# varunbachalli/PoseEstimationKF

Measured on AMD Instinct MI355X. Metric: EKF steps/sec (predict+Wahba+update) at batch=1M; HBM-roofline %, higher is better.
Workload: dtype f64

## Files before the change

### poseestimationkf_amd/csrc/pekf_math.hpp

```cpp
#pragma once

#include <hip/hip_runtime.h>

#include <cmath>
#include <cstdint>
#include <type_traits>

#define PEKF_DEV __device__ __forceinline__

#ifdef PEKF_ISA_COMMON_PATH
#define PEKF_TAKEN(cond, common) (common)
#else
#define PEKF_TAKEN(cond, common) __builtin_expect(!!(cond), 0)
#endif

namespace pekf {

constexpr double kNsToS = 1e-09;
constexpr double kSqrt2 = 1.4142135623730951;


PEKF_DEV void omega_half(const double *w, double *A) {
    A[0] = 0.0;          A[1] = -0.5 * w[0];  A[2] = -0.5 * w[1];  A[3] = -0.5 * w[2];
    A[4] = 0.5 * w[0];   A[5] = 0.0;          A[6] = 0.5 * w[2];   A[7] = -0.5 * w[1];
// ... 303 lines not shown
}

template <int FAST>
PEKF_DEV void wahba_current_rank1(const double *acc0, const double *mag0, const double *acc, const double *mag,
                                  double ka, double km, double *R) {
    double v[3], w[3];
    current_rank1_directions<FAST>(acc0, mag0, acc, mag, ka, km, v, w);
    shortest_arc<FAST>(v, w, R);
}

template <int FAST>
PEKF_DEV void wahba_current_rank1_quat(const double *acc0, const double *mag0, const double *acc, const double *mag,
                                       double ka, double km, double *q) {
    double v[3], w[3], n[3];
    current_rank1_directions<FAST>(acc0, mag0, acc, mag, ka, km, v, w);
    const double c1 = fma(v[0], w[0], fma(v[1], w[1], fma(v[2], w[2], 1.0)));
    const double k[3] = {v[1] * w[2] - v[2] * w[1], v[2] * w[0] - v[0] * w[2], v[0] * w[1] - v[1] * w[0]};
    normal_of(v, n);
    const bool half = !(c1 * c1 + k[0] * k[0] + k[1] * k[1] + k[2] * k[2] > 0.0) && (w[0] == w[0]);
    const double t[4] = {half ? 0.0 : c1, half ? n[0] : k[0], half ? n[1] : k[1], half ? n[2] : k[2]};
    const double it = rsqrt<FAST>(t[0] * t[0] + t[1] * t[1] + t[2] * t[2] + t[3] * t[3]);
    q[0] = t[0] * it; q[1] = t[1] * it; q[2] = t[2] * it; q[3] = t[3] * it;
}

PEKF_DEV void frame_pair(const Frame &F, double *a, double *m) {
#pragma unroll
    for (int i = 0; i < 3; ++i) {
        a[i] = F.alpha * F.e1[i];
        m[i] = F.beta1 * F.e1[i] + F.beta2 * F.e2[i];
    }
}

PEKF_DEV void wahba_rotation_vectors(const double *acc0, const double *mag0, const double *acc,
                                     const double *mag, double ka, double km, double *R) {
    Frame W, V;
    make_frame(acc0, mag0, W);
    make_frame(acc, mag, V, wahba_sign(ka, km));
    if (frame_degenerate(W) || frame_degenerate(V))
        wahba_rank1_rotation(acc0, mag0, acc, mag, ka, km, R);
    else
        wahba_rotation(W, V, ka, km, R);
}

PEKF_DEV void rotm_to_quat_scaled(const double *M, double *v, double &inv_s) {
    const double t1 = ((1.0 + M[0]) - M[4]) - M[8];
    const double t2 = ((1.0 - M[0]) + M[4]) - M[8];
    const double t3 = ((1.0 - M[0]) - M[4]) + M[8];
    const bool b1 = (t1 > t2) && (t1 > t3);
    const bool b2 = !b1 && (t2 > t1) && (t2 > t3);
    const bool b3 = !b1 && !b2;
    const double t = b1 ? t1 : (b2 ? t2 : t3);
    inv_s = 0.5 * rsqrt<true>(t);
    const double dw1 = M[7] - M[5], dw2 = M[2] - M[6], dw3 = M[3] - M[1];
    const double sxy = M[1] + M[3], sxz = M[2] + M[6], syz = M[5] + M[7];
    v[0] = b1 ? dw1 : (b2 ? dw2 : dw3);
    v[1] = b1 ? t : (b2 ? sxy : sxz);
    v[2] = b2 ? t : (b1 ? sxy : syz);
    v[3] = b3 ? t : (b1 ? sxz : syz);
}

PEKF_DEV void rotm_to_quat_fast(const double *M, double *q) {
    double v[4], inv_s;
    rotm_to_quat_scaled(M, v, inv_s);
    q[0] = v[0] * inv_s; q[1] = v[1] * inv_s; q[2] = v[2] * inv_s; q[3] = v[3] * inv_s;
}

PEKF_DEV void q4_times(const double *M, const double *z, double *v, double &nv, double &t0) {
    const double a = 1.0 + M[8], b = 1.0 - M[8], s = M[0] + M[4], d = M[0] - M[4];
    t0 = a + s;
    const double t1 = b + d, t2 = b - d, t3 = a - s;
    const double dw1 = M[7] - M[5], dw2 = M[2] - M[6], dw3 = M[3] - M[1];
    const double sxy = M[1] + M[3], sxz = M[2] + M[6], syz = M[5] + M[7];
    v[0] = fma(t0, z[0], fma(dw1, z[1], fma(dw2, z[2], dw3 * z[3])));
    v[1] = fma(dw1, z[0], fma(t1, z[1], fma(sxy, z[2], sxz * z[3])));
    v[2] = fma(dw2, z[0], fma(sxy, z[1], fma(t2, z[2], syz * z[3])));
    v[3] = fma(dw3, z[0], fma(sxz, z[1], fma(syz, z[2], t3 * z[3])));
    nv = fma(v[0], v[0], fma(v[1], v[1], fma(v[2], v[2], v[3] * v[3])));
}

PEKF_DEV void rotm_to_quat_flip_reference(const double *M, const double *z, double *v, double &sc) {
    double inv_s;
    rotm_to_quat_scaled(M, v, inv_s);
    const double cmp = v[0] * z[0] + v[1] * z[1] + v[2] * z[2] + v[3] * z[3];
    sc = cmp < 0.0 ? -inv_s : inv_s;
}

PEKF_DEV void rotm_to_quat_toward(const double *M, const double *z, double *v, double &sc) {
    double nv, t0;
    q4_times(M, z, v, nv, t0);
    sc = rsqrt<true>(nv);
    if (PEKF_TAKEN(nv < 1.0 || t0 > 4.0 - 1e-10, false))
        rotm_to_quat_flip_reference(M, z, v, sc);
}

struct RefW {
    static constexpr bool kRefBasis = true;
    double aW, b1W, b2W;
    double q[4];
    PEKF_DEV void quat(double *o) const { o[0] = q[0]; o[1] = q[1]; o[2] = q[2]; o[3] = q[3]; }
};

PEKF_DEV void frame_quat(const Frame &F, double *q) {
    const double m00 = F.e1[0], m10 = F.e1[1], m20 = F.e1[2];
    const double m01 = F.e2[0], m11 = F.e2[1], m21 = F.e2[2];
    const double m02 = F.u3[0], m12 = F.u3[1], m22 = F.u3[2];
    const double t0 = 1.0 + m00 + m11 + m22, t1 = 1.0 + m00 - m11 - m22;
    const double t2 = 1.0 - m00 + m11 - m22, t3 = 1.0 - m00 - m11 + m22;
    const double w1 = m21 - m12, w2 = m02 - m20, w3 = m10 - m01;
    const double sxy = m01 + m10, sxz = m02 + m20, syz = m12 + m21;
    double v0, v1, v2, v3;
    if (t0 >= t1 && t0 >= t2 && t0 >= t3) {
        v0 = t0; v1 = w1; v2 = w2; v3 = w3;
    } else if (t1 >= t2 && t1 >= t3) {
        v0 = w1; v1 = t1; v2 = sxy; v3 = sxz;
    } else if (t2 >= t3) {
        v0 = w2; v1 = sxy; v2 = t2; v3 = syz;
    } else {
        v0 = w3; v1 = sxz; v2 = syz; v3 = t3;
    }
    const double in = 1.0 / sqrt(v0 * v0 + v1 * v1 + v2 * v2 + v3 * v3);
    q[0] = v0 * in; q[1] = v1 * in; q[2] = v2 * in; q[3] = v3 * in;
}

struct RefWLazy {
    static constexpr bool kRefBasis = true;
    double aW, b1W, b2W;
    const double *pair;
    PEKF_DEV void quat(double *o) const {
        Frame F;
        make_frame<true>(pair, pair + 3, F);
        frame_quat(F, o);
    }
};

template <bool CONJ>
PEKF_DEV void qmul_left(const double *q, const double *x, double *y) {
    const double q0 = q[0], q1 = CONJ ? -q[1] : q[1], q2 = CONJ ? -q[2] : q[2], q3 = CONJ ? -q[3] : q[3];
    y[0] = q0 * x[0] - q1 * x[1] - q2 * x[2] - q3 * x[3];
    y[1] = q0 * x[1] + q1 * x[0] + q2 * x[3] - q3 * x[2];
    y[2] = q0 * x[2] - q1 * x[3] + q2 * x[0] + q3 * x[1];
    y[3] = q0 * x[3] + q1 * x[2] - q2 * x[1] + q3 * x[0];
}

PEKF_DEV void quat_to_rotm(const double *q, double *M) {
    const double w = q[0], x = q[1], y = q[2], z = q[3];
    M[0] = 1.0 - 2.0 * (y * y + z * z); M[1] = 2.0 * (x * y - w * z);       M[2] = 2.0 * (x * z + w * y);
    M[3] = 2.0 * (x * y + w * z);       M[4] = 1.0 - 2.0 * (x * x + z * z); M[5] = 2.0 * (y * z - w * x);
    M[6] = 2.0 * (x * z - w * y);       M[7] = 2.0 * (y * z + w * x);       M[8] = 1.0 - 2.0 * (x * x + y * y);
}

struct NoPin {
    PEKF_DEV void operator()() const {}
};
template <int F = 1, class RW, std::enable_if_t<RW::kRefBasis, int> = 0>
PEKF_DEV void wahba_rotation_ref(const RW &W, const Frame &V, double ka, double km, double *R) {
    const double kw = km * W.b2W, kb = km * W.b1W;
    double p = ka * W.aW * V.alpha + kb * V.beta1 + kw * V.beta2;
    double s = kw * V.beta1 - kb * V.beta2;
    const double ih = rsqrt<F>(p * p + s * s);
    p *= ih;
    s *= ih;
#pragma unroll
    for (int j = 0; j < 3; ++j) {
        R[j] = p * V.e1[j] - s * V.e2[j];
        R[3 + j] = s * V.e1[j] + p * V.e2[j];
        R[6 + j] = V.u3[j];
    }
}

template <int F = 1, class RW, class Reload, class Pin = NoPin, std::enable_if_t<RW::kRefBasis, int> = 0>
PEKF_DEV void wahba_toward_from_rotation(const RW &W, const double *R, const double *z, double *v, double &sc,
                                         const Reload &reload, const Pin &pin = Pin()) {
    double nv, t0;
    q4_times(R, z, v, nv, t0);
    sc = rsqrt<F>(nv);
    pin();
    if (PEKF_TAKEN(!(nv >= 1.0), false)) {
        double Fw[9], Rw[9], zw[4], vw[4], qw[4];
        W.quat(qw);
        quat_to_rotm(qw, Fw);
#pragma unroll
        for (int i = 0; i < 3; ++i)
#pragma unroll
            for (int j = 0; j < 3; ++j) Rw[3 * i + j] = Fw[3 * i] * R[j] + Fw[3 * i + 1] * R[3 + j] + Fw[3 * i + 2] * R[6 + j];
        qmul_left<false>(qw, z, zw);
        rotm_to_quat_flip_reference(Rw, zw, vw, sc);
        qmul_left<true>(qw, vw, v);
        if (!(nv == nv)) {
            double acc[3], mag[3];
            reload(acc, mag);
            const double a0[3] = {W.aW, 0.0, 0.0}, m0[3] = {W.b1W, W.b2W, 0.0}, kr = fabs(acc[2]);
            wahba_current_rank1_quat<1>(a0, m0, acc, mag, kr, 1.0 - kr, v);
            sc = v[0] * z[0] + v[1] * z[1] + v[2] * z[2] + v[3] * z[3] < 0.0 ? -1.0 : 1.0;
        }
    }
    (void)t0;
}

template <int F = 1, class RW, class Reload, class Pin = NoPin, std::enable_if_t<RW::kRefBasis, int> = 0>
PEKF_DEV void wahba_quat_toward(const RW &W, const Frame &V, double ka, double km, const double *z, double *v,
                                double &sc, const Reload &reload, const Pin &pin = Pin()) {
    const double kw = km * W.b2W, kb = km * W.b1W;
    double p = ka * W.aW * V.alpha + kb * V.beta1 + kw * V.beta2;
    double s = kw * V.beta1 - kb * V.beta2;
    const double ih = rsqrt<F>(p * p + s * s);
    p *= ih;
    s *= ih;
    double R[9];
#pragma unroll
    for (int j = 0; j < 3; ++j) {
        R[j] = p * V.e1[j] - s * V.e2[j];
        R[3 + j] = s * V.e1[j] + p * V.e2[j];
        R[6 + j] = V.u3[j];
    }
    double nv, t0;
    q4_times(R, z, v, nv, t0);
    sc = rsqrt<F>(nv);
    pin();
    if (PEKF_TAKEN(!(nv >= 1.0), false)) {
        double Fw[9], Rw[9], zw[4], vw[4], qw[4];
        W.quat(qw);
        quat_to_rotm(qw, Fw);
#pragma unroll
        for (int i = 0; i < 3; ++i)
#pragma unroll
            for (int j = 0; j < 3; ++j) Rw[3 * i + j] = Fw[3 * i] * R[j] + Fw[3 * i + 1] * R[3 + j] + Fw[3 * i + 2] * R[6 + j];
        qmul_left<false>(qw, z, zw);
        rotm_to_quat_flip_reference(Rw, zw, vw, sc);
        qmul_left<true>(qw, vw, v);
        if (!(nv == nv)) {
            double acc[3], mag[3];
            reload(acc, mag);
            const double a0[3] = {W.aW, 0.0, 0.0}, m0[3] = {W.b1W, W.b2W, 0.0}, kr = fabs(acc[2]);
            wahba_current_rank1_quat<1>(a0, m0, acc, mag, kr, 1.0 - kr, v);
            sc = v[0] * z[0] + v[1] * z[1] + v[2] * z[2] + v[3] * z[3] < 0.0 ? -1.0 : 1.0;
        }
    }
    (void)t0;
}

template <int F = 1, class Reload, class Pin = NoPin>
PEKF_DEV void wahba_quat_toward(const Frame &W, const Frame &V, double ka, double km, const double *z, double *v,
                                double &sc, const Reload &reload, const Pin & = Pin()) {
    double R[9], nv, t0;
    wahba_rotation<true>(W, V, ka, km, R);
    q4_times(R, z, v, nv, t0);
    sc = rsqrt<true>(nv);
    if (PEKF_TAKEN(!(nv >= 1.0) || t0 > 4.0 - 1e-10, false)) {
        rotm_to_quat_flip_reference(R, z, v, sc);
        if (!(nv == nv)) {
            double acc[3], mag[3], a0[3], m0[3];
            reload(acc, mag);
            frame_pair(W, a0, m0);
            const double kr = fabs(acc[2]);
            wahba_current_rank1_quat<1>(a0, m0, acc, mag, kr, 1.0 - kr, v);
            sc = v[0] * z[0] + v[1] * z[1] + v[2] * z[2] + v[3] * z[3] < 0.0 ? -1.0 : 1.0;
        }
    }
}


template <typename T>
struct Sym4T {
    T a00, a01, a02, a03, a11, a12, a13, a22, a23, a33;
};
using Sym4 = Sym4T<double>;

template <bool CONJ, typename T>
PEKF_DEV Sym4T<T> sym_rotate(const double *q, const Sym4T<T> &S) {
    const double p[4][4] = {{S.a00, S.a01, S.a02, S.a03}, {S.a01, S.a11, S.a12, S.a13},
                            {S.a02, S.a12, S.a22, S.a23}, {S.a03, S.a13, S.a23, S.a33}};
    double t[4][4], o[4][4];
#pragma unroll
    for (int j = 0; j < 4; ++j) {
        double c[4];
        qmul_left<CONJ>(q, p[j], c);
#pragma unroll
        for (int i = 0; i < 4; ++i) t[i][j] = c[i];
    }
#pragma unroll
    for (int i = 0; i < 4; ++i) qmul_left<CONJ>(q, t[i], o[i]);
    return {(T)o[0][0], (T)o[0][1], (T)o[0][2], (T)o[0][3], (T)o[1][1],
            (T)o[1][2], (T)o[1][3], (T)o[2][2], (T)o[2][3], (T)o[3][3]};
}

template <bool FAST>
PEKF_DEV float recip(float x) {
    if (!FAST) return 1.0f / x;
    float r = __builtin_amdgcn_rcpf(x);
    return fmaf(r, fmaf(-x, r, 1.0f), r);
}

template <typename T>
PEKF_DEV Sym4T<T> innovation_cov2(const Sym4T<T> &P, const T *h, const T *w, T th2, const T *x, T n2, T g2, T r2,
                                  T g2x) {
    const T sp = P.a00 + P.a11, dp = P.a11 - P.a00, sq = P.a22 + P.a33, dq = P.a22 - P.a33;
    const T tr = sp + sq, d11 = sq - sp, d22 = dp - dq, d33 = dp + dq;
    const T u0 = fma(d11, h[0], fma(P.a03 - P.a12, w[1], -(P.a02 + P.a13) * w[2]));
    const T u1 = fma(d22, h[1], fma(P.a01 - P.a23, w[2], -(P.a03 + P.a12) * w[0]));
    const T u2 = fma(d33, h[2], fma(P.a02 - P.a13, w[0], -(P.a01 + P.a23) * w[1]));
    const T uh = fma(u0, h[0], fma(u1, h[1], u2 * h[2]));
    const T c0 = fma(u1, h[2], -u2 * h[1]), c1 = fma(u2, h[0], -u0 * h[2]);
    const T c2 = fma(u0, h[1], -u1 * h[0]);
    const T nt = T(-2) * th2;
    const T base = fma(th2, tr, fma(g2, n2, r2));
    const T b0 = base - uh, bk = base + uh;
    const T gx0 = g2x * x[0], gx1 = g2x * x[1], gx2 = g2x * x[2], gx3 = g2x * x[3];
    Sym4T<T> o;
    o.a00 = fma(nt, P.a00, fma(-gx0, x[0], b0));
    o.a01 = fma(nt, P.a01, fma(-gx0, x[1], c0));
    o.a02 = fma(nt, P.a02, fma(-gx0, x[2], c1));
    o.a03 = fma(nt, P.a03, fma(-gx0, x[3], c2));
    o.a11 = fma(nt, P.a11, fma(-gx1, x[1], fma(-u0, w[0], bk)));
    o.a22 = fma(nt, P.a22, fma(-gx2, x[2], fma(-u1, w[1], bk)));
    o.a33 = fma(nt, P.a33, fma(-gx3, x[3], fma(-u2, w[2], bk)));
    o.a12 = fma(nt, P.a12, fma(-gx1, x[2], -fma(u0, h[1], u1 * h[0])));
    o.a13 = fma(nt, P.a13, fma(-gx1, x[3], -fma(u0, h[2], u2 * h[0])));
    o.a23 = fma(nt, P.a23, fma(-gx2, x[3], -fma(u1, h[2], u2 * h[1])));
    return o;
}

template <typename T>
PEKF_DEV Sym4T<T> innovation_cov_n(const Sym4T<T> &N, const T *h, const T *w, T th2, const T *x, T n2, T gb, T rb,
                                   T gbx) {
    const T sp = N.a00 + N.a11, dp = N.a11 - N.a00, sq = N.a22 + N.a33, dq = N.a22 - N.a33;
    const T tr = sp + sq, d11 = sq - sp, d22 = dp - dq, d33 = dp + dq;
    const T u0 = fma(d11, h[0], fma(N.a12 - N.a03, w[1], (N.a02 + N.a13) * w[2]));
    const T u1 = fma(d22, h[1], fma(N.a01 - N.a23, w[2], (N.a03 + N.a12) * w[0]));
    const T u2 = fma(d33, h[2], fma(N.a13 - N.a02, w[0], -(N.a01 + N.a23) * w[1]));
    const T uh = fma(u0, h[0], fma(u1, h[1], u2 * h[2]));
    const T c0 = fma(u1, h[2], -u2 * h[1]), c1 = fma(u2, h[0], -u0 * h[2]);
    const T c2 = fma(u0, h[1], -u1 * h[0]);
    const T nt = T(-2) * th2;
    const T base = fma(th2, tr + rb, fma(gb, n2, rb));
    const T b0 = base - uh, bk = base + uh;
    const T gx0 = gbx * x[0], gx1 = gbx * x[1], gx2 = gbx * x[2], gx3 = gbx * x[3];
    Sym4T<T> o;
    o.a00 = fma(nt, N.a00, fma(-gx0, x[0], b0));
    o.a01 = fma(nt, N.a01, fma(-gx0, x[1], c0));
    o.a02 = fma(-nt, N.a02, fma(-gx0, x[2], c1));
    o.a03 = fma(-nt, N.a03, fma(-gx0, x[3], c2));
    o.a11 = fma(nt, N.a11, fma(-gx1, x[1], fma(-u0, w[0], bk)));
    o.a22 = fma(nt, N.a22, fma(-gx2, x[2], fma(-u1, w[1], bk)));
    o.a33 = fma(nt, N.a33, fma(-gx3, x[3], fma(-u2, w[2], bk)));
    o.a12 = fma(-nt, N.a12, fma(-gx1, x[2], -fma(u0, h[1], u1 * h[0])));
    o.a13 = fma(-nt, N.a13, fma(-gx1, x[3], -fma(u0, h[2], u2 * h[0])));
    o.a23 = fma(nt, N.a23, fma(-gx2, x[3], -fma(u1, h[2], u2 * h[1])));
    return o;
}

PEKF_DEV Sym4 innovation_cov_n_w(const Sym4 &N, const double *w, double th2x2, const double *x, double n2, double gb,
                                 double rb, double rbh, double gbx) {
    const double sp = N.a00 + N.a11, dp = N.a11 - N.a00, sq = N.a22 + N.a33, dq = N.a22 - N.a33;
    const double trh = add_half(sp, sq) + rbh;
    const double d11h = sub_half(sq, sp), d22h = sub_half(dp, dq), d33h = add_half(dp, dq);
    const double u0 = fma(d11h, w[0], fma(N.a12 - N.a03, w[1], (N.a02 + N.a13) * w[2]));
    const double u1 = fma(d22h, w[1], fma(N.a01 - N.a23, w[2], (N.a03 + N.a12) * w[0]));
    const double u2 = fma(d33h, w[2], fma(N.a13 - N.a02, w[0], -(N.a01 + N.a23) * w[1]));
    const double uh = fma_half(u0, w[0], fma(u1, w[1], u2 * w[2]));
    const double c0 = fma_half_nc(u1, w[2], u2 * w[1]), c1 = fma_half_nc(u2, w[0], u0 * w[2]);
    const double c2 = fma_half_nc(u0, w[1], u1 * w[0]);
    const double base = fma(th2x2, trh, fma(gb, n2, rb));
    const double b0 = base - uh, bk = base + uh;
    const double gx0 = gbx * x[0], gx1 = gbx * x[1], gx2 = gbx * x[2], gx3 = gbx * x[3];
    Sym4 o;
    o.a00 = fma(-th2x2, N.a00, fma(-gx0, x[0], b0));
    o.a01 = fma(-th2x2, N.a01, fma(-gx0, x[1], c0));
    o.a02 = fma(th2x2, N.a02, fma(-gx0, x[2], c1));
    o.a03 = fma(th2x2, N.a03, fma(-gx0, x[3], c2));
    o.a11 = fma(-th2x2, N.a11, fma(-gx1, x[1], fma(-u0, w[0], bk)));
    o.a22 = fma(-th2x2, N.a22, fma(-gx2, x[2], fma(-u1, w[1], bk)));
    o.a33 = fma(-th2x2, N.a33, fma(-gx3, x[3], fma(-u2, w[2], bk)));
    o.a12 = fma(th2x2, N.a12, fma(-gx1, x[2], -fma_half(u0, w[1], u1 * w[0])));
    o.a13 = fma(th2x2, N.a13, fma(-gx1, x[3], -fma_half(u0, w[2], u2 * w[0])));
    o.a23 = fma(-th2x2, N.a23, fma(-gx2, x[3], -fma_half(u1, w[2], u2 * w[1])));
    return o;
}

template <typename T, bool FAST = true, bool NEG = false>
PEKF_DEV Sym4T<T> spd_inverse_schur(const Sym4T<T> &S) {
    const T ia = recip<FAST>(S.a00 * S.a11 - S.a01 * S.a01);
    const T p00 = S.a11 * ia, p01 = -S.a01 * ia, p11 = S.a00 * ia;
    const T x00 = p00 * S.a02 + p01 * S.a12, x01 = p00 * S.a03 + p01 * S.a13;
    const T x10 = p01 * S.a02 + p11 * S.a12, x11 = p01 * S.a03 + p11 * S.a13;
    const T c00 = S.a22 - S.a02 * x00 - S.a12 * x10;
    const T c01 = S.a23 - S.a02 * x01 - S.a12 * x11;
    const T c11 = S.a33 - S.a03 * x01 - S.a13 * x11;
    const T ic = NEG ? recip<FAST>(c01 * c01 - c00 * c11) : recip<FAST>(c00 * c11 - c01 * c01);
    const T q00 = c11 * ic, q01 = -c01 * ic, q11 = c00 * ic;
    Sym4T<T> o;
    if (NEG) {
// ... 67 lines not shown
```

### poseestimationkf_amd/csrc/pekf_step.hpp

```cpp
#pragma once

#include <type_traits>

#include "pekf_internal.hpp"
#include "pekf_math.hpp"
#include "pekf_tile.hpp"

namespace pekf {

constexpr int kRunBlock = 256;

#ifndef PEKF_REC_AUX
#define PEKF_REC_AUX 2
#endif

template <bool SOA, typename PT>
__device__ __forceinline__ void load_state(const double *X, const double *P, int64_t b, int64_t batch,
                                           double *x, Sym4T<PT> &S) {
    if (SOA) {
#pragma unroll
        for (int k = 0; k < 4; ++k) x[k] = X[k * batch + b];
        S = {(PT)P[0 * batch + b], (PT)P[1 * batch + b], (PT)P[2 * batch + b], (PT)P[3 * batch + b],
             (PT)P[4 * batch + b], (PT)P[5 * batch + b], (PT)P[6 * batch + b], (PT)P[7 * batch + b],
             (PT)P[8 * batch + b], (PT)P[9 * batch + b]};
// ... 40 lines not shown

    __device__ __forceinline__ RowCursor(const float4 *gd, const float4 *am, const float2 *my, int64_t batch,
                                         int64_t win)
        : g(reinterpret_cast<const char *>(gd)), a(reinterpret_cast<const char *>(am)),
          m(reinterpret_cast<const char *>(my)), row16((uint32_t)batch * 16u), row8((uint32_t)batch * 8u),
          window((int32_t)win) {
        const uint32_t c = (1u << 31) / row16;
        chunk_rows = c ? (int32_t)c : 1;
    }
    __device__ __forceinline__ void start(int32_t r) {
        row = r;
        end = (window - r < chunk_rows) ? window : r + chunk_rows;
        const uint64_t n = (uint64_t)(end - r);
        rg = row_rsrc(g + (uint64_t)r * row16, (int64_t)(n * row16));
        ra = row_rsrc(a + (uint64_t)r * row16, (int64_t)(n * row16));
        rm = row_rsrc(m + (uint64_t)r * row8, (int64_t)(n * row8));
        s16 = 0;
        s8 = 0;
    }
    __device__ __forceinline__ void advance() {
        if (++row == end) {
            start(row == window ? 0 : row);
        } else {
            s16 += row16;
            s8 += row8;
        }
    }
    __device__ __forceinline__ Rec load(uint32_t off16, uint32_t off8) const {
        Rec v;
        v.gd = __builtin_bit_cast(float4, __builtin_amdgcn_raw_buffer_load_b128(rg, off16, s16, PEKF_REC_AUX));
        v.am = __builtin_bit_cast(float4, __builtin_amdgcn_raw_buffer_load_b128(ra, off16, s16, PEKF_REC_AUX));
        v.my = __builtin_bit_cast(float2, __builtin_amdgcn_raw_buffer_load_b64(rm, off8, s8, PEKF_REC_AUX));
        return v;
    }
};

template <typename PT>
__device__ __forceinline__ Sym4T<PT> sym_from16(const double (&p)[16]) {
    return {(PT)p[0], (PT)p[1], (PT)p[2], (PT)p[3], (PT)p[5], (PT)p[6], (PT)p[7], (PT)p[10], (PT)p[11], (PT)p[15]};
}
template <typename PT>
__device__ __forceinline__ void sym_to16(const Sym4T<PT> &S, double (&p)[16]) {
    p[0] = S.a00; p[1] = S.a01; p[2] = S.a02; p[3] = S.a03;
    p[4] = S.a01; p[5] = S.a11; p[6] = S.a12; p[7] = S.a13;
    p[8] = S.a02; p[9] = S.a12; p[10] = S.a22; p[11] = S.a23;
    p[12] = S.a03; p[13] = S.a13; p[14] = S.a23; p[15] = S.a33;
}

__device__ __forceinline__ double state_norm2(const double *x) {
    const double n2 = x[0] * x[0] + x[1] * x[1] + x[2] * x[2] + x[3] * x[3];
    return fabs(n2 - 1.0) < 1e-13 ? 1.0 : n2;
}

__device__ __forceinline__ double fma_sub(double a, double b, double c) {
    double d;
    asm("v_fma_f64 %0, %1, %2, -%3" : "=v"(d) : "v"(a), "v"(b), "v"(c));
    return d;
}
__device__ __forceinline__ double fma_rsub(double a, double b, double c) {
    double d;
    asm("v_fma_f64 %0, -%1, %2, %3" : "=v"(d) : "v"(a), "v"(b), "v"(c));
    return d;
}

template <typename PT>
struct StepK {
    PT g2, r2;
    PT rp, rr;
    double sy;
};
template <typename PT, bool MC>
__device__ __forceinline__ StepK<PT> step_consts(double qs, double rs) {
    const double g = 0.25 * qs;
    if (MC) {
        const double ib = 1.0 / (kSqrt2 * rs);
        return {(PT)(2.0 * g * ib), (PT)(2.0 * rs * ib), (PT)(rs * ib), PT(0), 1.0 / kSqrt2};
    }
    return {(PT)(2.0 * g), (PT)(2.0 * rs), (PT)rs, (PT)(2.0 * (rs * rs)), 0.5 / rs};
}

template <typename PT, bool MC>
__device__ __forceinline__ void record_skip(double *x, const double *z, Sym4T<PT> &P, const Sym4T<PT> &S2,
                                            const StepK<PT> &k) {
    x[0] = z[0]; x[1] = z[1]; x[2] = z[2]; x[3] = z[3];
    const PT hf = PT(0.5);
    if (MC)
        P = {fma(hf, S2.a00, -k.r2), hf * S2.a01, -hf * S2.a02, -hf * S2.a03, fma(hf, S2.a11, -k.r2),
             -hf * S2.a12, -hf * S2.a13, fma(hf, S2.a22, -k.r2), hf * S2.a23, fma(hf, S2.a33, -k.r2)};
    else
        P = {fma(hf, S2.a00, -k.rp), hf * S2.a01, hf * S2.a02, hf * S2.a03, fma(hf, S2.a11, -k.rp),
             hf * S2.a12, hf * S2.a13, fma(hf, S2.a22, -k.rp), hf * S2.a23, fma(hf, S2.a33, -k.rp)};
}

template <typename PT, bool MC>
__device__ __forceinline__ void record_correct(double *x, const double *z, Sym4T<PT> &P, const Sym4T<PT> &Si,
                                               const double *v, double sc, const StepK<PT> &k) {
    const PT e0 = (PT)fma_sub(v[0], sc, z[0]), e1 = (PT)fma_sub(v[1], sc, z[1]);
    const PT e2 = (PT)(MC ? fma_rsub(v[2], sc, z[2]) : fma_sub(v[2], sc, z[2]));
    const PT e3 = (PT)(MC ? fma_rsub(v[3], sc, z[3]) : fma_sub(v[3], sc, z[3]));
    const double u0 = Si.a00 * e0 + Si.a01 * e1 + Si.a02 * e2 + Si.a03 * e3;
    const double u1 = Si.a01 * e0 + Si.a11 * e1 + Si.a12 * e2 + Si.a13 * e3;
    const double u2 = Si.a02 * e0 + Si.a12 * e1 + Si.a22 * e2 + Si.a23 * e3;
    const double u3 = Si.a03 * e0 + Si.a13 * e1 + Si.a23 * e2 + Si.a33 * e3;
    const double sr = sc * k.sy;
    const double x0 = fma(v[0], sr, MC ? u0 : -u0), x1 = fma(v[1], sr, MC ? u1 : -u1);
    const double x2 = fma(v[2], sr, -u2), x3 = fma(v[3], sr, -u3);
    if (MC) {
        x[0] = x0; x[1] = x1; x[2] = x2; x[3] = x3;
    } else {
        const double in = rsqrt<true>(x0 * x0 + x1 * x1 + x2 * x2 + x3 * x3);
        x[0] = x0 * in; x[1] = x1 * in; x[2] = x2 * in; x[3] = x3 * in;
    }
    if (MC) {
        P = Si;
    } else {
        const PT rp = k.rp, rr = k.rr;
        P = {rp - rr * Si.a00, -rr * Si.a01, -rr * Si.a02, -rr * Si.a03, rp - rr * Si.a11,
             -rr * Si.a12, -rr * Si.a13, rp - rr * Si.a22, -rr * Si.a23, rp - rr * Si.a33};
    }
}

template <typename PT, bool MC = false, bool LAZY = false, bool OM = false, bool PIN = false, bool HOIST = false,
          typename Ref, typename Reload>
__device__ __forceinline__ void ekf_record_step(double *x, double n2, Sym4T<PT> &P, const Ref &Wf, const StepK<PT> &k,
                                                const double *gy, double dt_ns, bool missing,
                                                const double *acc, const double *mag, const Reload &reload) {
    static_assert(!OM || (MC && std::is_same<PT, double>::value), "omod form: FP64 multi-record loop only");
    static_assert(!HOIST || OM, "hoisted form: FP64 multi-record loop only");
    constexpr int F = OM ? 2 : 1;
    const double n2x = LAZY ? x[0] * x[0] + x[1] * x[1] + x[2] * x[2] + x[3] * x[3] : n2;
    double z[4], kk, irk;
    Sym4T<PT> S2;
    if constexpr (OM) {
        const double th2x2 = fma_half(gy[2], gy[2], fma(gy[1], gy[1], gy[0] * gy[0]));
        rk4_closed_w(x, n2x, dt_ns, gy, th2x2, z, kk, irk);
        const double g2x = LAZY ? ((irk * irk) * kk) * k.g2 : k.g2;
        S2 = innovation_cov_n_w(P, gy, th2x2, x, LAZY ? 1.0 : n2, k.g2, k.r2, k.rp, g2x);
    } else {
        const double hw[3] = {0.5 * gy[0], 0.5 * gy[1], 0.5 * gy[2]};
        const double th2 = hw[0] * hw[0] + hw[1] * hw[1] + hw[2] * hw[2];
        const PT hp[3] = {(PT)hw[0], (PT)hw[1], (PT)hw[2]};
        const PT wp[3] = {(PT)gy[0], (PT)gy[1], (PT)gy[2]};
        const PT xp[4] = {(PT)x[0], (PT)x[1], (PT)x[2], (PT)x[3]};
        rk4_closed(x, n2x, dt_ns, hw, th2, z, kk, irk);
        const PT g2x = LAZY ? (PT)((irk * irk) * kk) * k.g2 : k.g2;
        const PT n2p = LAZY ? PT(1) : (PT)n2;
        S2 = MC ? innovation_cov_n<PT>(P, hp, wp, (PT)th2, xp, n2p, k.g2, k.r2, g2x)
                : innovation_cov2<PT>(P, hp, wp, (PT)th2, xp, n2p, k.g2, k.r2, g2x);
    }

    if constexpr (HOIST) {
        const Sym4T<PT> Si = spd_inverse_schur<PT, true, MC>(S2);
        const double ka = fabs(acc[2]);
        Frame Vf;
        make_frame<F>(acc, mag, Vf, 1.0 - ka);
        double R[9];
        wahba_rotation_ref<F>(Wf, Vf, ka, 1.0 - ka, R);
        asm volatile("" ::"v"(Si.a00), "v"(Si.a01), "v"(Si.a02), "v"(Si.a03), "v"(Si.a11), "v"(Si.a12),
                     "v"(Si.a13), "v"(Si.a22), "v"(Si.a23), "v"(Si.a33), "v"(R[0]), "v"(R[1]), "v"(R[2]),
                     "v"(R[3]), "v"(R[4]), "v"(R[5]), "v"(R[6]), "v"(R[7]), "v"(R[8]));
        if (missing) {
            record_skip<PT, MC>(x, z, P, S2, k);
        } else {
            double v[4], sc;
            wahba_toward_from_rotation<F>(Wf, R, z, v, sc, reload);
            record_correct<PT, MC>(x, z, P, Si, v, sc, k);
        }
        return;
    }
    if (missing) {
        x[0] = z[0]; x[1] = z[1]; x[2] = z[2]; x[3] = z[3];
        const PT hf = PT(0.5);
        if (MC)
            P = {fma(hf, S2.a00, -k.r2), hf * S2.a01, -hf * S2.a02, -hf * S2.a03, fma(hf, S2.a11, -k.r2),
                 -hf * S2.a12, -hf * S2.a13, fma(hf, S2.a22, -k.r2), hf * S2.a23, fma(hf, S2.a33, -k.r2)};
        else
            P = {fma(hf, S2.a00, -k.rp), hf * S2.a01, hf * S2.a02, hf * S2.a03, fma(hf, S2.a11, -k.rp),
                 hf * S2.a12, hf * S2.a13, fma(hf, S2.a22, -k.rp), hf * S2.a23, fma(hf, S2.a33, -k.rp)};
    } else {
        const Sym4T<PT> Si = spd_inverse_schur<PT, true, MC>(S2);

        const double ka = fabs(acc[2]);
        Frame Vf;
        make_frame<F>(acc, mag, Vf, 1.0 - ka);
        double v[4], sc;
        auto pin = [&] {
            if constexpr (PIN && MC && OM)
                asm volatile("" ::"v"(Si.a00), "v"(Si.a01), "v"(Si.a02), "v"(Si.a03), "v"(Si.a11), "v"(Si.a12),
                             "v"(Si.a13), "v"(Si.a22), "v"(Si.a23), "v"(Si.a33));
        };
        wahba_quat_toward<F>(Wf, Vf, ka, 1.0 - ka, z, v, sc, reload, pin);
        const PT e0 = (PT)fma_sub(v[0], sc, z[0]), e1 = (PT)fma_sub(v[1], sc, z[1]);
        const PT e2 = (PT)(MC ? fma_rsub(v[2], sc, z[2]) : fma_sub(v[2], sc, z[2]));
        const PT e3 = (PT)(MC ? fma_rsub(v[3], sc, z[3]) : fma_sub(v[3], sc, z[3]));
        const double u0 = Si.a00 * e0 + Si.a01 * e1 + Si.a02 * e2 + Si.a03 * e3;
        const double u1 = Si.a01 * e0 + Si.a11 * e1 + Si.a12 * e2 + Si.a13 * e3;
        const double u2 = Si.a02 * e0 + Si.a12 * e1 + Si.a22 * e2 + Si.a23 * e3;
        const double u3 = Si.a03 * e0 + Si.a13 * e1 + Si.a23 * e2 + Si.a33 * e3;
        const double sr = sc * k.sy;
        const double x0 = fma(v[0], sr, MC ? u0 : -u0), x1 = fma(v[1], sr, MC ? u1 : -u1);
        const double x2 = fma(v[2], sr, -u2), x3 = fma(v[3], sr, -u3);
        if (MC) {
            x[0] = x0; x[1] = x1; x[2] = x2; x[3] = x3;
        } else {
            const double in = rsqrt<true>(x0 * x0 + x1 * x1 + x2 * x2 + x3 * x3);
            x[0] = x0 * in; x[1] = x1 * in; x[2] = x2 * in; x[3] = x3 * in;
        }
        if (MC) {
            P = Si;
        } else {
            const PT rp = k.rp, rr = k.rr;
            P = {rp - rr * Si.a00, -rr * Si.a01, -rr * Si.a02, -rr * Si.a03, rp - rr * Si.a11,
                 -rr * Si.a12, -rr * Si.a13, rp - rr * Si.a22, -rr * Si.a23, rp - rr * Si.a33};
        }
    }
}

template <typename PT>
__device__ __forceinline__ void to_ref_basis(const double *qw, double *x, Sym4T<PT> &P, double rs) {
    double xw[4];
    qmul_left<true>(qw, x, xw);
    x[0] = xw[0]; x[1] = xw[1]; x[2] = xw[2]; x[3] = xw[3];
    P = sym_rotate<true>(qw, P);
    const PT ib = (PT)(1.0 / (kSqrt2 * rs)), rp = (PT)rs;
    P = {(P.a00 - rp) * ib, P.a01 * ib, -P.a02 * ib, -P.a03 * ib, (P.a11 - rp) * ib,
         -P.a12 * ib, -P.a13 * ib, (P.a22 - rp) * ib, P.a23 * ib, (P.a33 - rp) * ib};
}
template <typename PT, typename RW>
__device__ __forceinline__ void from_ref_basis(const RW &Wr, double *x, Sym4T<PT> &P, double rs) {
    const PT be = (PT)(kSqrt2 * rs), rp = (PT)rs;
    P = {fma(be, P.a00, rp), be * P.a01, -be * P.a02, -be * P.a03, fma(be, P.a11, rp),
         -be * P.a12, -be * P.a13, fma(be, P.a22, rp), be * P.a23, fma(be, P.a33, rp)};
    const double in = rsqrt<true>(x[0] * x[0] + x[1] * x[1] + x[2] * x[2] + x[3] * x[3]);
    const double xn[4] = {x[0] * in, x[1] * in, x[2] * in, x[3] * in};
    double xo[4], qw[4];
    Wr.quat(qw);
    qmul_left<false>(qw, xn, xo);
    x[0] = xo[0]; x[1] = xo[1]; x[2] = xo[2]; x[3] = xo[3];
    P = sym_rotate<false>(qw, P);
}

#ifndef PEKF_RUN_WAVES
#define PEKF_RUN_WAVES 0
#endif
#if PEKF_RUN_WAVES
#define PEKF_RUN_ATTR __attribute__((amdgpu_waves_per_eu(PEKF_RUN_WAVES)))
#else
#define PEKF_RUN_ATTR
#endif

template <bool TRAJ, bool MIXED, bool SOA, bool COUNTS, bool ONE, bool PIN = false, bool LONGDT = false,
          bool HOIST = false>
__global__ __launch_bounds__(kRunBlock) PEKF_RUN_ATTR void k_run(int64_t batch, int64_t n_steps, int64_t window,
                                                   int64_t step0, const float4 *__restrict__ gd,
                                                   const float4 *__restrict__ am,
                                                   const float2 *__restrict__ my,
                                                   const double *__restrict__ refs,
                                                   double *__restrict__ Xio, double *__restrict__ Pio,
                                                   double qs, double rs, double *__restrict__ traj,
                                                   const int32_t *__restrict__ counts,
                                                   const double *__restrict__ dtx) {
    using PT = typename std::conditional<MIXED, float, double>::type;
    if constexpr (ONE) {
        constexpr int kTile = SOA ? 6 : 16;
        __shared__ double pool[kRunBlock / kWave * tile_doubles<kTile>()];
        const WaveTile t(pool, tile_doubles<kTile>(), batch);
        double cx[4], cp[16], cr[6];
        if constexpr (!SOA) {
            t.gather(Xio, cx);
            t.gather(Pio, cp);
        }
        t.gather(refs, cr);
        const bool act = t.active();
        const uint32_t lane = act ? (uint32_t)(t.first + t.lane) : 0u;
        const int64_t base = (step0 % window) * batch;
        const Rec cur = {(gd + base)[lane], (am + base)[lane], (my + base)[lane]};
        const bool run = act && (!COUNTS || counts[lane] > 0);
        double x[4], pv[16], rf[6];
        Sym4T<PT> P;
        if constexpr (SOA) {
            load_state<true>(Xio, Pio, lane, batch, x, P);
        } else {
            t.to_lanes(cx, x);
            t.to_lanes(cp, pv);
            P = sym_from16<PT>(pv);
        }
        t.to_lanes(cr, rf);
        Frame Wf;
        make_frame<true>(rf, rf + 3, Wf);
        if (run) {
            const double gy[3] = {cur.gd.x, cur.gd.y, cur.gd.z};
            const uint32_t word = __float_as_uint(cur.gd.w);
            const double acc[3] = {cur.am.x, cur.am.y, cur.am.z};
            const double mag[3] = {cur.am.w, cur.my.x, cur.my.y};
            double dtn = (double)(word & PEKF_DT_MASK);
            if constexpr (LONGDT) {
                if ((word & PEKF_DT_MASK) == PEKF_DT_ESCAPE) dtn = (dtx + base)[lane];
            }
            auto reload = [&](double *a, double *m) {
                const float4 va = (am + base)[lane];
                const float2 vm = (my + base)[lane];
                a[0] = va.x; a[1] = va.y; a[2] = va.z;
                m[0] = va.w; m[1] = vm.x; m[2] = vm.y;
            };
            ekf_record_step<PT>(x, state_norm2(x), P, Wf, step_consts<PT, false>(qs, rs), gy, dtn,
                                (word & PEKF_MISSING_MAG_BIT) != 0, acc, mag, reload);
        }
        if (TRAJ && act) {
            double2 *o = reinterpret_cast<double2 *>(traj) + 2 * (int64_t)lane;
            o[0] = make_double2(x[0], x[1]);
            o[1] = make_double2(x[2], x[3]);
        }
        if constexpr (SOA) {
            if (act) store_state<true>(Xio, Pio, lane, batch, x, P);
        } else {
            sym_to16(P, pv);
            t.store(Xio, x);
            t.store(Pio, pv);
        }
        return;
    }
    const int64_t b = (int64_t)blockIdx.x * kRunBlock + threadIdx.x;
    if (b >= batch) return;
    const int32_t my_steps = COUNTS ? (counts[b] < n_steps ? counts[b] : (int32_t)n_steps) : (int32_t)n_steps;

    Frame Wf;
    {
        const double a0[3] = {refs[6 * b + 0], refs[6 * b + 1], refs[6 * b + 2]};
        const double m0[3] = {refs[6 * b + 3], refs[6 * b + 4], refs[6 * b + 5]};
        make_frame<true>(a0, m0, Wf);
    }
    double x[4];
    Sym4T<PT> P;
    load_state<SOA>(Xio, Pio, b, batch, x, P);

    const uint32_t lane = (uint32_t)b;
    const uint32_t off16 = lane * 16u, off8 = lane * 8u;
    RowCursor rows(gd, am, my, batch, window);
    constexpr int32_t kLag = 1;
    auto step = [&](const Rec &cur, int32_t t, double n2, const auto &ref, auto lazy) {
        constexpr bool MC = !std::is_same<std::decay_t<decltype(ref)>, Frame>::value;
        if (!COUNTS || t < my_steps) {
            const double gy[3] = {cur.gd.x, cur.gd.y, cur.gd.z};
            const uint32_t word = __float_as_uint(cur.gd.w);
// ... 80 lines not shown
```

Before: 82.95 billion.

## Compute Wahba quaternion directly from vector products instead of rotation matrix

Replaces the frame construction, 3x3 rotation matrix build and matrix-to-quaternion step in the Wahba solve with a closed-form unnormalized quaternion built straight from the accelerometer and magnetometer products. The sign and scale toward the prior quaternion come from a single dot product and rsqrt. The old matrix path is kept as a rare fallback, which reloads the inputs and is taken when alignment is poor or the weight is negative. This cuts FP64 arithmetic and register pressure in the update step, at the cost of more branching and possible numerical differences near the branch thresholds.

```diff
diff --git a/poseestimationkf_amd/csrc/pekf_math.hpp b/poseestimationkf_amd/csrc/pekf_math.hpp
--- a/poseestimationkf_amd/csrc/pekf_math.hpp
+++ b/poseestimationkf_amd/csrc/pekf_math.hpp
@@ -479,30 +479,34 @@
 struct NoPin {
     PEKF_DEV void operator()() const {}
 };
-template <int F = 1, class RW, std::enable_if_t<RW::kRefBasis, int> = 0>
-PEKF_DEV void wahba_rotation_ref(const RW &W, const Frame &V, double ka, double km, double *R) {
+template <int F = 1, class RW, class Reload, std::enable_if_t<RW::kRefBasis, int> = 0>
+PEKF_DEV void wahba_matrix_toward(const RW &W, const Reload &reload, const double *z, double *v, double &sc) {
+    Frame V;
+    double ka, km;
+    {
+        double acc[3], mag[3];
+        reload(acc, mag);
+        ka = fabs(acc[2]);
+        km = 1.0 - ka;
+        make_frame<F>(acc, mag, V, km);
+    }
     const double kw = km * W.b2W, kb = km * W.b1W;
     double p = ka * W.aW * V.alpha + kb * V.beta1 + kw * V.beta2;
     double s = kw * V.beta1 - kb * V.beta2;
     const double ih = rsqrt<F>(p * p + s * s);
     p *= ih;
     s *= ih;
+    double R[9];
 #pragma unroll
     for (int j = 0; j < 3; ++j) {
         R[j] = p * V.e1[j] - s * V.e2[j];
         R[3 + j] = s * V.e1[j] + p * V.e2[j];
         R[6 + j] = V.u3[j];
     }
-}
-
-template <int F = 1, class RW, class Reload, class Pin = NoPin, std::enable_if_t<RW::kRefBasis, int> = 0>
-PEKF_DEV void wahba_toward_from_rotation(const RW &W, const double *R, const double *z, double *v, double &sc,
-                                         const Reload &reload, const Pin &pin = Pin()) {
     double nv, t0;
     q4_times(R, z, v, nv, t0);
     sc = rsqrt<F>(nv);
-    pin();
-    if (PEKF_TAKEN(!(nv >= 1.0), false)) {
+    if (!(nv >= 1.0)) {
         double Fw[9], Rw[9], zw[4], vw[4], qw[4];
         W.quat(qw);
         quat_to_rotm(qw, Fw);
@@ -524,46 +528,54 @@
     (void)t0;
 }
 
+template <int F = 1, class RW, std::enable_if_t<RW::kRefBasis, int> = 0>
+PEKF_DEV void wahba_product_ref(const RW &W, const double *a, const double *m, double ka, double km, double *q) {
+    const double sa = a[0] * a[0] + a[1] * a[1] + a[2] * a[2];
+    const double ias = copysign(rsqrt<F>(sa), a[0]);
+    const double nas = sa * ias;
+    const double ws = nas + a[0];
+    const double b1s = (a[0] * m[0] + a[1] * m[1] + a[2] * m[2]) * ias;
+    const double us = b1s + m[0];
+    const double tys = ws * m[1] - a[1] * us;
+    const double ntz = a[2] * us - ws * m[2];
+    const double sb = tys * tys + ntz * ntz;
+    const double hs = sb * copysign(rsqrt<F>(sb), a[0]);
+    const double kw = km * W.b2W, kb = km * W.b1W;
+    const double aw = fabs(nas) * ws, b1w = b1s * fabs(ws);
+    const double p = ka * W.aW * aw + kb * b1w + kw * hs;
+    const double s = kw * b1w - kb * hs;
+    const double n = p * p + s * s;
+    const double h = n * rsqrt<F>(n);
+    const double wt = h + fabs(p), wb = fabs(hs) + fabs(tys);
+    const bool ft = p >= 0.0, fb = tys >= 0.0;
+    const double c0 = ft ? wt : s, c3 = ft ? s : wt;
+    const double b0 = fb ? wb : ntz, b1 = fb ? ntz : wb;
+    const double r0 = b0 * ws, r1 = b1 * ws, r2 = b0 * a[2] + b1 * a[1], r3 = b1 * a[2] - b0 * a[1];
+    q[0] = c0 * r0 - c3 * r3;
+    q[1] = c0 * r1 - c3 * r2;
+    q[2] = c0 * r2 + c3 * r1;
+    q[3] = c0 * r3 + c3 * r0;
+}
+
 template <int F = 1, class RW, class Reload, class Pin = NoPin, std::enable_if_t<RW::kRefBasis, int> = 0>
-PEKF_DEV void wahba_quat_toward(const RW &W, const Frame &V, double ka, double km, const double *z, double *v,
-                                double &sc, const Reload &reload, const Pin &pin = Pin()) {
-    const double kw = km * W.b2W, kb = km * W.b1W;
-    double p = ka * W.aW * V.alpha + kb * V.beta1 + kw * V.beta2;
-    double s = kw * V.beta1 - kb * V.beta2;
-    const double ih = rsqrt<F>(p * p + s * s);
-    p *= ih;
-    s *= ih;
-    double R[9];
-#pragma unroll
-    for (int j = 0; j < 3; ++j) {
-        R[j] = p * V.e1[j] - s * V.e2[j];
-        R[3 + j] = s * V.e1[j] + p * V.e2[j];
-        R[6 + j] = V.u3[j];
-    }
-    double nv, t0;
-    q4_times(R, z, v, nv, t0);
-    sc = rsqrt<F>(nv);
+PEKF_DEV void wahba_toward_from_product(const RW &W, const double *q, double km, const double *z,
+                                        double *v, double &sc, const Reload &reload, const Pin &pin = Pin()) {
+    const double c = fma(q[0], z[0], fma(q[1], z[1], fma(q[2], z[2], q[3] * z[3])));
+    const double nq = fma(q[0], q[0], fma(q[1], q[1], fma(q[2], q[2], q[3] * q[3])));
+    sc = copysign(rsqrt<F>(nq), c);
+    v[0] = q[0]; v[1] = q[1]; v[2] = q[2]; v[3] = q[3];
     pin();
-    if (PEKF_TAKEN(!(nv >= 1.0), false)) {
-        double Fw[9], Rw[9], zw[4], vw[4], qw[4];
-        W.quat(qw);
-        quat_to_rotm(qw, Fw);
-#pragma unroll
-        for (int i = 0; i < 3; ++i)
-#pragma unroll
-            for (int j = 0; j < 3; ++j) Rw[3 * i + j] = Fw[3 * i] * R[j] + Fw[3 * i + 1] * R[3 + j] + Fw[3 * i + 2] * R[6 + j];
-        qmul_left<false>(qw, z, zw);
-        rotm_to_quat_flip_reference(Rw, zw, vw, sc);
-        qmul_left<true>(qw, vw, v);
-        if (!(nv == nv)) {
-            double acc[3], mag[3];
-            reload(acc, mag);
-            const double a0[3] = {W.aW, 0.0, 0.0}, m0[3] = {W.b1W, W.b2W, 0.0}, kr = fabs(acc[2]);
-            wahba_current_rank1_quat<1>(a0, m0, acc, mag, kr, 1.0 - kr, v);
-            sc = v[0] * z[0] + v[1] * z[1] + v[2] * z[2] + v[3] * z[3] < 0.0 ? -1.0 : 1.0;
-        }
-    }
-    (void)t0;
+    if (PEKF_TAKEN(!(c * sc >= 0.25) || !(km >= 0.0), false)) {
+        wahba_matrix_toward<F>(W, reload, z, v, sc);
+    }
+}
+
+template <int F = 1, class RW, class Reload, class Pin = NoPin, std::enable_if_t<RW::kRefBasis, int> = 0>
+PEKF_DEV void wahba_quat_toward(const RW &W, const double *acc, const double *mag, double ka, double km,
+                                const double *z, double *v, double &sc, const Reload &reload, const Pin &pin = Pin()) {
+    double q[4];
+    wahba_product_ref<F>(W, acc, mag, ka, km, q);
+    wahba_toward_from_product<F>(W, q, km, z, v, sc, reload, pin);
 }
 
 template <int F = 1, class Reload, class Pin = NoPin>
diff --git a/poseestimationkf_amd/csrc/pekf_step.hpp b/poseestimationkf_amd/csrc/pekf_step.hpp
--- a/poseestimationkf_amd/csrc/pekf_step.hpp
+++ b/poseestimationkf_amd/csrc/pekf_step.hpp
@@ -216,18 +216,16 @@
     if constexpr (HOIST) {
         const Sym4T<PT> Si = spd_inverse_schur<PT, true, MC>(S2);
         const double ka = fabs(acc[2]);
-        Frame Vf;
-        make_frame<F>(acc, mag, Vf, 1.0 - ka);
-        double R[9];
-        wahba_rotation_ref<F>(Wf, Vf, ka, 1.0 - ka, R);
+        double qm[4];
+        wahba_product_ref<F>(Wf, acc, mag, ka, 1.0 - ka, qm);
         asm volatile("" ::"v"(Si.a00), "v"(Si.a01), "v"(Si.a02), "v"(Si.a03), "v"(Si.a11), "v"(Si.a12),
-                     "v"(Si.a13), "v"(Si.a22), "v"(Si.a23), "v"(Si.a33), "v"(R[0]), "v"(R[1]), "v"(R[2]),
-                     "v"(R[3]), "v"(R[4]), "v"(R[5]), "v"(R[6]), "v"(R[7]), "v"(R[8]));
+                     "v"(Si.a13), "v"(Si.a22), "v"(Si.a23), "v"(Si.a33), "v"(qm[0]), "v"(qm[1]), "v"(qm[2]),
+                     "v"(qm[3]));
         if (missing) {
             record_skip<PT, MC>(x, z, P, S2, k);
         } else {
             double v[4], sc;
-            wahba_toward_from_rotation<F>(Wf, R, z, v, sc, reload);
+            wahba_toward_from_product<F>(Wf, qm, 1.0 - ka, z, v, sc, reload);
             record_correct<PT, MC>(x, z, P, Si, v, sc, k);
         }
         return;
@@ -245,15 +243,19 @@
         const Sym4T<PT> Si = spd_inverse_schur<PT, true, MC>(S2);
 
         const double ka = fabs(acc[2]);
-        Frame Vf;
-        make_frame<F>(acc, mag, Vf, 1.0 - ka);
         double v[4], sc;
         auto pin = [&] {
             if constexpr (PIN && MC && OM)
                 asm volatile("" ::"v"(Si.a00), "v"(Si.a01), "v"(Si.a02), "v"(Si.a03), "v"(Si.a11), "v"(Si.a12),
                              "v"(Si.a13), "v"(Si.a22), "v"(Si.a23), "v"(Si.a33));
         };
-        wahba_quat_toward<F>(Wf, Vf, ka, 1.0 - ka, z, v, sc, reload, pin);
+        if constexpr (std::is_same<Ref, Frame>::value) {
+            Frame Vf;
+            make_frame<F>(acc, mag, Vf, 1.0 - ka);
+            wahba_quat_toward<F>(Wf, Vf, ka, 1.0 - ka, z, v, sc, reload, pin);
+        } else {
+            wahba_quat_toward<F>(Wf, acc, mag, ka, 1.0 - ka, z, v, sc, reload, pin);
+        }
         const PT e0 = (PT)fma_sub(v[0], sc, z[0]), e1 = (PT)fma_sub(v[1], sc, z[1]);
         const PT e2 = (PT)(MC ? fma_rsub(v[2], sc, z[2]) : fma_sub(v[2], sc, z[2]));
         const PT e3 = (PT)(MC ? fma_rsub(v[3], sc, z[3]) : fma_sub(v[3], sc, z[3]));
```

New measurement: 87.43 billion (median of 6 runs). 5.4% higher.
